# jmloveyj/ros_navigation

Measured on AMD Instinct MI355X. Metric: replan cycles/sec (HIMM+VFH++A*) on 4096x4096 grid, higher is better.
Workload: dtype int32

## Files before the change

### ros_navigation_amd/csrc/astar.hip

```cpp
#include "engine.hpp"

#include <algorithm>
#include <cfloat>
#include <cmath>
#include <cstdlib>
#include <cstring>
#include <chrono>
#include <thread>
#include <vector>

using namespace rna;

namespace {

constexpr int COST_D = 1414;

struct HostTrace {
  bool on = getenv("RNA_HOST_TRACE") != nullptr;
  double us[8] = {};
  long n = 0, queries = 0;
  std::chrono::steady_clock::time_point t;
  void start() { if (on) t = std::chrono::steady_clock::now(); }
  void lap(int k) {
    if (!on) return;
    const auto now = std::chrono::steady_clock::now();
    us[k] += std::chrono::duration<double, std::micro>(now - t).count();
    t = now;
  }
  void dump() {
    if (!on || n == 0) return;
    fprintf(stderr, "[host trace] %ld pipelined launches, us each: wait for a free stage %.1f (%.2f hipEventQuery calls) | ring entry's old batch %.1f | "
            "enqueue (events, snapshot, launch order, search, flag copy) %.1f | done event + bookkeeping %.1f\n", n, us[0] / n, (double)queries / n,
            us[1] / n, us[2] / n, us[3] / n);
    for (double& v : us) v = 0;
    n = 0; queries = 0;
  }
};
HostTrace g_trace;
struct StageTrace {
  hipEvent_t a[AstarDevice::MAX_DEPTH] = {}, c[AstarDevice::MAX_DEPTH] = {};
  std::chrono::steady_clock::time_point t_enq[AstarDevice::MAX_DEPTH];
  bool armed[AstarDevice::MAX_DEPTH] = {};
  double gpu_ms = 0, host_busy_ms = 0;
  long n = 0;
};
StageTrace g_stage;
void stage_trace_dump() {
  if (g_stage.n) fprintf(stderr, "[host trace] a stage's cycle, ms: from enqueue to the end of the search and what follows it on the stream %.2f (the search itself: roofline.avg_launch_ms) | "
                         "host: enqueue -> noticed free %.2f (%ld cycles)\n", g_stage.gpu_ms / g_stage.n, g_stage.host_busy_ms / g_stage.n, g_stage.n);
  g_stage.gpu_ms = g_stage.host_busy_ms = 0; g_stage.n = 0;
}

#define RNA_TRY(call) do { const int rc_try_ = (call); if (rc_try_ != RNA_OK) return rc_try_; } while (0)

int alloc_stage(rna_engine* e, int d) {
  AstarDevice& a = e->astar;
  AstarStage& s = a.stage[d];
  RNA_TRY(dev_alloc(e, &s.pool, tsa_pool_bytes(a.max_queries, a.page_cap) / sizeof(unsigned)));
  RNA_TRY(dev_alloc(e, &s.rev, (size_t)a.rev_cap * a.max_queries));
  RNA_TRY(dev_alloc(e, &s.block, tsa_stage_bytes(e)));
  RNA_HIP(e, hipMemsetAsync(s.block, 0, tsa_stage_bytes(e), e->stream));
  RNA_TRY(tsa_stage_prepare(e, d));
  if (a.page_cap < tsa_tiles(e)) {
    RNA_TRY(dev_alloc(e, &s.retry_pool, tsa_retry_pool_bytes(e) / sizeof(unsigned)));
    RNA_TRY(dev_alloc(e, &s.retry_block, tsa_retry_bytes(e)));
    RNA_HIP(e, hipMemsetAsync(s.retry_block, 0, tsa_retry_bytes(e), e->stream));
    RNA_TRY(tsa_retry_prepare(e, d));
  }
  if (a.depth == 1) return RNA_OK;
  int prio_lo = 0, prio_hi = 0;
  (void)hipDeviceGetStreamPriorityRange(&prio_lo, &prio_hi);
  if (getenv("RNA_NO_STREAM_PRIORITY")) prio_lo = prio_hi = 0;
  int skip = e->cu_count / 8;
  if (const char* m = getenv("RNA_SEARCH_CU_SKIP")) skip = atoi(m);
  if (skip > 0 && skip < e->cu_count) {
    uint32_t mask[16] = {};
    const int words = (e->cu_count + 31) / 32 < 16 ? (e->cu_count + 31) / 32 : 16;
    for (int c = skip; c < e->cu_count && c < 512; ++c) mask[c >> 5] |= 1u << (c & 31);
    RNA_HIP(e, hipExtStreamCreateWithCUMask(&s.stream, (uint32_t)words, mask));
  } else {
    RNA_HIP(e, hipStreamCreateWithPriority(&s.stream, hipStreamNonBlocking, prio_lo));
  }
  RNA_HIP(e, hipEventCreateWithFlags(&s.done, hipEventDisableTiming));
  RNA_HIP(e, hipEventCreateWithFlags(&s.snap_done, hipEventDisableTiming));
  return RNA_OK;
}

void free_stage(AstarStage& s) {
  dev_free(&s.pool); dev_free(&s.rev); dev_free(&s.block); dev_free(&s.retry_pool); dev_free(&s.retry_block);
  if (s.stream) (void)hipStreamDestroy(s.stream);
  if (s.done) (void)hipEventDestroy(s.done);
  if (s.snap_done) (void)hipEventDestroy(s.snap_done);
  s = AstarStage{};
}

int alloc_stages_impl(rna_engine* e) {
  AstarDevice& a = e->astar;
  for (int d = 0; d < a.depth; ++d) RNA_TRY(alloc_stage(e, d));
  if (a.depth > 1) {
    RNA_HIP(e, hipEventCreateWithFlags(&a.ev_init, hipEventDisableTiming));
    RNA_HIP(e, hipEventCreateWithFlags(&a.ev_prep, hipEventDisableTiming));
    a.ring_n = 2 * a.depth;
    a.ring_stride = tsa_ring_bytes(e);
    RNA_TRY(dev_alloc(e, &a.ring_mem, a.ring_stride * (size_t)a.ring_n));
    RNA_HIP(e, hipMemsetAsync(a.ring_mem, 0, a.ring_stride * (size_t)a.ring_n, e->stream));
    for (int r = 0; r < a.ring_n; ++r) RNA_HIP(e, hipEventCreateWithFlags(&a.ring[r].free, hipEventDisableTiming));
  }
  if (a.stage[0].retry_pool) {
    RNA_HIP(e, hipHostMalloc(reinterpret_cast<void**>(&a.retry_flag), AstarDevice::MAX_DEPTH * sizeof(int), hipHostMallocCoherent));
    for (int d = 0; d < AstarDevice::MAX_DEPTH; ++d) a.retry_flag[d] = 0;
    for (int d = 0; d < a.depth; ++d) a.stage[d].retry_flag = a.retry_flag + d;
  }
  a.launches = 0;
  RNA_TRY(dev_alloc(e, &a.queries_dev, (size_t)a.max_queries));
  RNA_TRY(dev_alloc(e, &a.results_dev, (size_t)a.max_queries));
  return RNA_OK;
}

int alloc_stages(rna_engine* e) {
  const int rc = alloc_stages_impl(e);
  if (rc != RNA_OK) {
    const std::string why = e->err;
    (void)astar_release(e);
    e->err = why;
  }
  return rc;
}

int ensure_config(rna_engine* e) {
  AstarDevice& a = e->astar;
  if (a.live()) return RNA_OK;
// ... 334 lines not shown
```

### ros_navigation_amd/csrc/astar_tile.hip

```cpp
#include "engine.hpp"
#include <algorithm>
#include <cstring>
#include <vector>

using namespace rna;

namespace rna {

constexpr int TI = 64, TJ = 16;
constexpr int TILE_WORDS = TI * TJ;
constexpr int AUX_WORDS = 64;
constexpr int MASK_STRIDE = TILE_WORDS + 32 + 128;
constexpr int TSA_WAVES = 8;
constexpr int TSA_WAVES_PER_EU = 8;
constexpr int TSA_HPASS = 4;
constexpr int TSA_IDLE_SLEEP = 4;
constexpr int TSA_PRIO_FIRST = 0;
constexpr int TSA_BT_PRIO = 3;
constexpr int TSA_SCOPE = __HIP_MEMORY_SCOPE_AGENT;
constexpr int TSA_MAX_TILE_WORDS = 2048;
constexpr int COST_S = 1000, COST_D = 1414;
constexpr int INF = 0x7fffffff;
constexpr int KU = 0x40000000;
constexpr int SCR_CNT = 84 + 192 + 48 + 64;
// ... 63 lines not shown
  return r;
}
__device__ __forceinline__ int tsa_octile24(int i, int j, int gi, int gj) {
  const int dx = abs(i - gi), dy = abs(j - gj);
  return tsa_h24(max(dx, dy), min(dx, dy));
}
__device__ __forceinline__ int tsa_prop(int u, int h, int thr) { return (u - h >= thr) ? u : 0; }

__device__ __forceinline__ int tile_of(int i, int j, int tiles_i) { return (j >> 4) * tiles_i + (i >> 6); }
__device__ __forceinline__ int in_page(int i, int j) { return ((j & 15) << 6) + (i & 63); }
__device__ __forceinline__ int kdi_of(int k) { return (k == 0 || k == 3 || k == 5) ? -1 : ((k == 2 || k == 4 || k == 7) ? 1 : 0); }
__device__ __forceinline__ int kdj_of(int k) { return k < 3 ? -1 : (k > 4 ? 1 : 0); }

struct TsaStage {
  unsigned* pages;
  unsigned* paux;
  unsigned* tmap;
  unsigned* owner;
  int* nalloc;
  uint8_t* nbr_tm;
  int* perm;
  int* ticket;
  int cap;
};
__host__ __device__ inline size_t tsa_align256(size_t x) { return (x + 255) & ~(size_t)255; }
constexpr int TSA_COUNTER_WORDS = 16;
__host__ __device__ inline unsigned long long* tsa_counters_of(const TsaStage& S) {
  return reinterpret_cast<unsigned long long*>(reinterpret_cast<char*>(S.nalloc) - TSA_COUNTER_WORDS * sizeof(unsigned long long));
}

__global__ void __launch_bounds__(256) tsa_snapshot_kernel(const uint8_t* __restrict__ nbr, int rows, int cols, int tiles_i, int tiles_j,
                                                             uint8_t* __restrict__ nbr_tm, int s0, int s1) {
  __shared__ unsigned s_free[256];
  const int a = threadIdx.x & 63, bq = threadIdx.x >> 6;
  for (int t = blockIdx.x; t < tiles_i * tiles_j; t += gridDim.x) {
    const int i = (t % tiles_i) * TI + a, j0 = (t / tiles_i) * TJ + bq * 4;
    unsigned v = 0u;
    if (i < rows) {
      const int bi = i + s0 >= rows ? i + s0 - rows : i + s0;
#pragma unroll
      for (int k = 0; k < 4; ++k)
        if (j0 + k < cols) {
          const int bj = j0 + k + s1 >= cols ? j0 + k + s1 - cols : j0 + k + s1;
          v |= (unsigned)nbr[(size_t)bj * rows + bi] << (8 * k);
        }
    }
    uint8_t* out = nbr_tm + (size_t)t * MASK_STRIDE;
    reinterpret_cast<unsigned*>(out)[a * 4 + bq] = v;
    if (a == 0) reinterpret_cast<unsigned*>(out + TILE_WORDS)[bq] = v;
    if (a == TI - 1) reinterpret_cast<unsigned*>(out + TILE_WORDS + 16)[bq] = v;
    s_free[threadIdx.x] = (((v & 0xffu) != 0u) ? 1u : 0u) | (((v & 0xff00u) != 0u) ? 2u : 0u) | (((v & 0xff0000u) != 0u) ? 4u : 0u) |
                          (((v & 0xff000000u) != 0u) ? 8u : 0u);
    __syncthreads();
    if (bq == 0)
      reinterpret_cast<unsigned short*>(out + TILE_WORDS + 32)[a] =
          (unsigned short)(s_free[a] | (s_free[64 + a] << 4) | (s_free[128 + a] << 8) | (s_free[192 + a] << 12));
    __syncthreads();
  }
}
__global__ void __launch_bounds__(256) tsa_prepare_kernel(TsaStage S, const rna_astar_query* __restrict__ queries, int n, int rows, int cols,
                                                          int ranked, int* __restrict__ served) {
  extern __shared__ int s_key[];
  if (threadIdx.x == 0) *S.ticket = 0;
  if (served && threadIdx.x < TSA_RETRY) served[threadIdx.x] = -1;
  if (served && threadIdx.x == TSA_RETRY) served[TSA_RETRY] = 0;
  if (!ranked) {
    for (int i = threadIdx.x; i < n; i += blockDim.x) S.perm[i] = i;
    return;
  }
  const int ncell = rows * cols;
  for (int i = threadIdx.x; i < n; i += blockDim.x) {
    const rna_astar_query q = queries[i];
    int key = -1;
    if (q.start >= 0 && q.goal >= 0 && q.start < ncell && q.goal < ncell) {
      const int di = abs(q.start % rows - q.goal % rows), dj = abs(q.start / rows - q.goal / rows);
      key = di > dj ? di : dj;
    }
    s_key[i] = key;
  }
  __syncthreads();
  for (int i = threadIdx.x; i < n; i += blockDim.x) {
    const int ki = s_key[i];
    int rank = 0;
    for (int j = 0; j < n; ++j) {
      const int kj = s_key[j];
      rank += (kj > ki || (kj == ki && j < i)) ? 1 : 0;
    }
    S.perm[rank] = i;
  }
}
__global__ void __launch_bounds__(256) tsa_zero_page0_kernel(unsigned* __restrict__ pages, unsigned* __restrict__ paux, int cap) {
  static_assert(TILE_WORDS / 4 == 256 && AUX_WORDS / 4 <= 256, "one uint4 of page 0 per thread");
  const size_t page0 = (size_t)blockIdx.x * ((size_t)cap + 1);
  reinterpret_cast<uint4*>(pages + (page0 << 10))[threadIdx.x] = make_uint4(0u, 0u, 0u, 0u);
  if (threadIdx.x < AUX_WORDS / 4) reinterpret_cast<uint4*>(paux + page0 * AUX_WORDS)[threadIdx.x] = make_uint4(0u, 0u, 0u, 0u);
// ... 884 lines not shown
    return;
  }
  asm volatile("s_waitcnt vmcnt(0)" ::: "memory");
  __builtin_amdgcn_wave_barrier();
  int32_t* path = A.paths + (size_t)q * A.max_path_len;
  for (int i = lane; i < len; i += 64) path[i] = tsa_buffer_lin(rev[len - 1 - i], rows, cols, A.s0, A.s1);
  if (lane == 0) A.results[q] = rna_astar_result{0, len, r.cost, r.expanded, r.rounds, r.buckets};
}

template <int WAVES, bool RETRY>
__global__ void __launch_bounds__(WAVES * 64) __attribute__((amdgpu_waves_per_eu(TSA_WAVES_PER_EU, TSA_WAVES_PER_EU))) tsa_search_kernel(const TsaLaunch A) {
  constexpr int TSA_THREADS = WAVES * 64;
  __shared__ __attribute__((aligned(16))) unsigned s_scr[WAVES][SCR_WORDS];
  extern __shared__ unsigned s_dyn[];
  __shared__ __attribute__((aligned(16))) unsigned s_node[TSA_NP];
  __shared__ __attribute__((aligned(16))) unsigned s_head[TSA_NCLS];
  __shared__ unsigned s_bm[TSA_BMW];
  __shared__ unsigned s_qc[TSA_QC];
  __shared__ int s_best, s_state, s_bucket, s_bucket0, s_jobs_done, s_jobs_noop, s_jobs_sticky, s_expanded, s_nalloc, s_any;
  __shared__ int s_count, s_spill, s_idle, s_open_left, s_open_pos, s_reruns;

  __shared__ int s_q, s_rank;
  if (!RETRY) {
    if (threadIdx.x == 0) { const int k = atomicAdd(A.S.ticket, 1); s_rank = k; s_q = A.S.perm[k]; }
  } else {
    if (threadIdx.x == 0) { s_q = A.retry_list[A.retry_base + (int)blockIdx.x]; s_rank = 1 << 30; }
  }
  __syncthreads();
  const int q = __builtin_amdgcn_readfirstlane(s_q);
  if (q < 0) return;
  if (RETRY && threadIdx.x == 0) A.S2.ticket[8 + blockIdx.x] = q;
  const TsaStage& S = RETRY ? A.S2 : A.S;
  const int sl = RETRY ? (int)blockIdx.x : q;
  if (__builtin_amdgcn_readfirstlane(s_rank) < A.prio_first) __builtin_amdgcn_s_setprio(3);
  const int tid = threadIdx.x, lane = tid & 63, wv = __builtin_amdgcn_readfirstlane(tid >> 6);
#ifdef RNA_TSA_STATS
  const unsigned long long t_kernel0 = wall_clock64();
#endif
  const int rows = A.rows, cols = A.cols, tiles_i = A.tiles_i, tiles_j = A.tiles_j;
  rna_astar_query qu = A.queries[q];
  const int ncell = rows * cols;
  const int ntile = tiles_i * tiles_j;
  const int nt_words = (ntile + 31) >> 5;
  unsigned* const s_st2 = s_dyn;
  unsigned* const s_open = s_dyn + 2 * nt_words;
  unsigned* const s_far = s_dyn + 3 * nt_words;
  rna_astar_result* const results = A.results;

  const bool valid = qu.start >= 0 && qu.goal >= 0 && qu.start < ncell && qu.goal < ncell;
  if (!valid) {
    if (tid == 0) results[q] = rna_astar_result{2, 0, INF, 0, 0, 0};
    return;
  }
  qu.start = tsa_unwrap_lin(qu.start, rows, cols, A.s0, A.s1);
  qu.goal = tsa_unwrap_lin(qu.goal, rows, cols, A.s0, A.s1);
  const int si = qu.start % rows, sj = qu.start / rows;
  const int gi = qu.goal % rows, gj = qu.goal / rows;

  TsaCtx C;
  C.rows = rows; C.cols = cols; C.tiles_i = tiles_i; C.tiles_j = tiles_j;
  C.tiles_magic = tiles_i > 1 ? (unsigned)(0x100000000ull / (unsigned)tiles_i) + 1u : 0u;
  C.pages = S.pages + (((size_t)sl * ((size_t)S.cap + 1)) << 10);
  C.paux = S.paux + (size_t)sl * ((size_t)S.cap + 1) * AUX_WORDS;
  C.tmap = S.tmap + (size_t)sl * ntile;
  C.owner = S.owner + (size_t)sl * (S.cap + 1);
  C.cap = S.cap;
  C.nalloc = &s_nalloc;
// ... 373 lines not shown
  const TsaGrid G = tsa_grid(e);
  KernelTimer kt(e, RNA_K_ASTAR_INIT, st);
  hipLaunchKernelGGL(tsa_snapshot_kernel, dim3(std::min(G.ti * G.tj, 4096)), dim3(256), 0, st, e->nbr, G.rows, G.cols, G.ti, G.tj,
                     tsa_launch_view(e, d, ring).nbr_tm, e->geom.start[0], e->geom.start[1]);
  RNA_HIP(e, hipGetLastError());
  return RNA_OK;
}
int tsa_order(rna_engine* e, int d, int ring, hipStream_t st, const rna_astar_query* q_dev, int n) {
  const TsaGrid G = tsa_grid(e);
  KernelTimer kt(e, RNA_K_ASTAR_RESET, st);
  const int ranked = n <= 2048 ? 1 : 0;
  hipLaunchKernelGGL(tsa_prepare_kernel, dim3(1), dim3(256), ranked ? (size_t)n * sizeof(int) : 0, st, tsa_launch_view(e, d, ring), q_dev, n, G.rows,
                     G.cols, ranked, tsa_retry_served(e, d));
  RNA_HIP(e, hipGetLastError());
  return RNA_OK;
}
int tsa_search(rna_engine* e, int d, int ring, hipStream_t st, const rna_astar_query* q_dev, int n, int32_t* paths_dev, int max_len,
               rna_astar_result* res_dev) {
  AstarDevice& a = e->astar;
  AstarStage& s = a.stage[d];
  const TsaGrid G = tsa_grid(e);
  const TsaStage S = tsa_launch_view(e, d, ring);
  KernelTimer kt(e, RNA_K_ASTAR_SEARCH, st);
  const size_t nt_bytes = (size_t)((G.ti * G.tj + 31) / 32) * sizeof(unsigned);
  TsaLaunch A;
  memset(&A, 0, sizeof(A));
  A.rows = G.rows; A.cols = G.cols; A.tiles_i = G.ti; A.tiles_j = G.tj; A.s0 = e->geom.start[0]; A.s1 = e->geom.start[1];
  A.queries = q_dev; A.S = S; A.bucket_width = a.bucket_width; A.paths = paths_dev; A.max_path_len = max_len;
  A.rev_all = s.rev; A.rev_cap = a.rev_cap; A.results = res_dev;
  A.retry = 0; A.n = n; A.S2 = S;
  A.prio_first = a.depth > 1 ? TSA_PRIO_FIRST : 0;
  if (const char* pf = getenv("RNA_TSA_PRIO_FIRST")) A.prio_first = atoi(pf);
  size_t lds_dyn = 4 * nt_bytes;
  if (const char* pad = getenv("RNA_TSA_LDS_PAD")) lds_dyn += (size_t)atoi(pad);
  const bool can_retry = s.retry_flag != nullptr;
  A.retry_count = can_retry ? tsa_retry_count(e, d) : nullptr;
  A.retry_list = can_retry ? tsa_retry_list(e, d) : nullptr;
  A.retry_base = 0;
  static const bool wide_env = getenv("RNA_TSA_WIDE") != nullptr;
  const bool wide = wide_env || n <= 32;
  if (a.depth > 1 && !wide) hipLaunchKernelGGL((tsa_search_kernel<TSA_WAVES, false>), dim3(n), dim3(TSA_WAVES * 64), lds_dyn, st, A);
  else hipLaunchKernelGGL((tsa_search_kernel<16, false>), dim3(n), dim3(16 * 64), lds_dyn, st, A);
  RNA_HIP(e, hipGetLastError());
  memcpy(s.last_launch, &A, sizeof(A));
  s.last_lds = lds_dyn;
  s.last_retried = 0;
  s.retry_armed = can_retry;
  return RNA_OK;
}

int tsa_counters_read(rna_engine* e, unsigned long long* out, bool reset) {
  AstarDevice& a = e->astar;
  for (int k = 0; k < TSA_COUNTER_WORDS; ++k) out[k] = 0ull;
  for (int d = 0; d < AstarDevice::MAX_DEPTH; ++d) {
    for (int view = 0; view < 2; ++view) {
      char* base = view ? a.stage[d].retry_block : a.stage[d].block;
      if (!base) continue;
      unsigned long long w[TSA_COUNTER_WORDS];
      char* cnt = base + TSA_HEAD_COUNTERS;
      RNA_HIP(e, hipMemcpyAsync(w, cnt, sizeof(w), hipMemcpyDeviceToHost, e->stream));
      if (reset) RNA_HIP(e, hipMemsetAsync(cnt, 0, sizeof(w), e->stream));
      RNA_HIP(e, hipStreamSynchronize(e->stream));
      for (int k = 0; k < TSA_COUNTER_WORDS; ++k) out[k] += w[k];
    }
  }
  return RNA_OK;
// ... 43 lines not shown
```

### ros_navigation_amd/csrc/engine.hip

```cpp
#include "engine.hpp"
#include "map_tiles_dev.hpp"

#include <cmath>
#include <dirent.h>
#include <unistd.h>
#include <cstdlib>
#include <cstring>
#include <limits>

using namespace rna;

__global__ void fill_f32_kernel(float* __restrict__ p, size_t n, float v) {
  size_t i = (size_t)blockIdx.x * blockDim.x + threadIdx.x;
  const size_t stride = (size_t)gridDim.x * blockDim.x;
  for (; i < n; i += stride) p[i] = v;
}

__global__ void compose_dirty_tiles_kernel(float* __restrict__ master, const float* __restrict__ laser,
                                           const unsigned* __restrict__ dirty, int rows, int cols, int tiles_i) {
  const int ti = blockIdx.x, tj = blockIdx.y;
  const int t = tj * tiles_i + ti;
  if (!reinterpret_cast<const unsigned char*>(dirty)[t]) return;
  const int i0 = ti * TILE, j0 = tj * TILE;
  const int li = threadIdx.x & (TILE - 1);
// ... 5 lines not shown
    }
  }
}

__global__ void nbr_mask_tiles_kernel(uint8_t* __restrict__ nbr, const float* __restrict__ master,
                                      const unsigned* __restrict__ dirty, int all, int rows, int cols,
                                      int tiles_i, int tiles_j, int s0, int s1) {
  const int ti = blockIdx.x, tj = blockIdx.y;
  if (!all && !dirty_ring(dirty, ti, tj, tiles_i, tiles_j)) return;
  __shared__ uint8_t blk[(TILE + 2) * (TILE + 2)];
  const int i0 = ti * TILE - 1, j0 = tj * TILE - 1;
  for (int k = threadIdx.x; k < (TILE + 2) * (TILE + 2); k += blockDim.x) {
    const int ii = k % (TILE + 2), jj = k / (TILE + 2);
    const int i = i0 + ii, j = j0 + jj;
    uint8_t b = 1;
    if (i >= 0 && j >= 0 && i < rows && j < cols) {
      b = cell_blocked(master[buffer_lin(i, j, rows, cols, s0, s1)]) ? 1 : 0;
    }
    blk[k] = b;
  }
  __syncthreads();
  for (int k = threadIdx.x; k < TILE * TILE; k += blockDim.x) {
    const int li = k & (TILE - 1), lj = k >> 6;
    const int i = ti * TILE + li, j = tj * TILE + lj;
    if (i >= rows || j >= cols) continue;
    nbr[buffer_lin(i, j, rows, cols, s0, s1)] = (uint8_t)nbr_mask_of(&blk[(lj + 1) * (TILE + 2) + (li + 1)], TILE + 2);
  }
}

__global__ void __launch_bounds__(256) compose_nbr_tiles_kernel(uint8_t* __restrict__ nbr, float* __restrict__ master, const float* __restrict__ laser,
                                                                const unsigned* __restrict__ dirty, unsigned* __restrict__ next_dirty, int rows,
                                                                int cols, int tiles_i, int tiles_j) {
  __shared__ uint8_t blk[(TILE + 2) * (TILE + 2)];
  for (int tt = blockIdx.x; tt < tiles_i * tiles_j; tt += gridDim.x)
    compose_nbr_tile(blk, tt, nbr, master, laser, dirty, next_dirty, rows, cols, tiles_i, tiles_j);
}

__global__ void clear_region_kernel(float* __restrict__ p, int rows, int i0, int ni, int j0, int nj) {
  const size_t n = (size_t)ni * nj;
  size_t k = (size_t)blockIdx.x * blockDim.x + threadIdx.x;
  const size_t stride = (size_t)gridDim.x * blockDim.x;
  const float nanv = __int_as_float(0x7fc00000);
  for (; k < n; k += stride) {
    const int i = i0 + (int)(k % ni), j = j0 + (int)(k / ni);
    p[(size_t)j * rows + i] = nanv;
  }
}

__global__ void __launch_bounds__(256) pack_tiles_kernel(const float* __restrict__ layer, int rows, int tiles_i,
                                                         const int32_t* __restrict__ tiles, int wi0, int wi1, int wj0,
                                                         int wj1, float* __restrict__ dense) {
  const int t = tiles[blockIdx.x];
  const int i0 = (t % tiles_i) * TILE, j0 = (t / tiles_i) * TILE;
  float* out = dense + (size_t)blockIdx.x * (TILE * TILE);
  for (int k = threadIdx.x; k < TILE * TILE; k += 256) {
    const int i = i0 + (k & (TILE - 1)), j = j0 + (k >> 6);
    out[k] = (i >= wi0 && i < wi1 && j >= wj0 && j < wj1) ? layer[(size_t)j * rows + i] : 0.0f;
  }
}

__global__ void __launch_bounds__(256) unpack_tiles_kernel(float* __restrict__ layer_a, float* __restrict__ layer_b,
                                                           int rows, int tiles_i, const int32_t* __restrict__ tiles,
                                                           int wi0, int wi1, int wj0, int wj1,
                                                           const float* __restrict__ dense,
                                                           unsigned* __restrict__ dirty_tiles) {
  const int t = tiles[blockIdx.x];
// ... 689 lines not shown
```

### ros_navigation_amd/csrc/engine.hpp

```cpp
#pragma once

#include <hip/hip_runtime.h>

#include <cstdint>
#include <cstdio>
#include <string>
#include <vector>

#include "../../include/rna.h"
#include "gridmath.hpp"
#include "map_state.hpp"

namespace {
struct GfCtl;
struct FrCtl;
}

namespace rna {

constexpr int TILE = 64;

struct HimmSlot { int cell; int head; int len; int offset; };

struct HimmScratch {
  int cap_rays = 0;
  int n_slots = 0;
  rna_ray* rays_dev = nullptr;
  int4* desc = nullptr;
  int* ncells = nullptr;
  int* next = nullptr;
  HimmSlot* slots = nullptr;
  int* seqs = nullptr;
  unsigned* before = nullptr;
  unsigned* after = nullptr;
  int* total = nullptr;
  unsigned* mark_bitmap = nullptr;
  int* pairs = nullptr;
  size_t pairs_cap = 0;
  bool pairs_checked = false;
  int* pairs_total_host = nullptr;
  int* tile_bins = nullptr;
  int win[4] = {0, 0, 0, 0};
};

struct VfhDevice {
  bool ready = false;
  rna_vfh_params p{};
  int n_robots = 0;
  int W = 0, H = 0, T = 0, CX = 0, CY = 0, NQ = 0, NQF = 0, NW = 0, max_speed = 0;
  float *cell_dist = nullptr, *cell_base_mag = nullptr, *cell_dir = nullptr;
  int* range_idx = nullptr;
  unsigned* memb = nullptr;
  unsigned* in_circle = nullptr;
// ... 7 lines not shown
};

struct AstarStage {
  unsigned* pool = nullptr;
  int32_t* rev = nullptr;
  char* block = nullptr;
  unsigned* retry_pool = nullptr;
  char* retry_block = nullptr;
  hipStream_t stream = nullptr;
  hipEvent_t done = nullptr;
  hipEvent_t snap_done = nullptr;
  bool snap_pending = false;
  bool busy = false;
  unsigned long long seq = 0;
  int* retry_flag = nullptr;
  bool retry_armed = false;
  int last_retried = 0;
  size_t last_lds = 0;
  alignas(8) unsigned char last_launch[384] = {};
};
struct AstarRingEntry {
  hipEvent_t free = nullptr;
  bool used = false;
};

struct AstarDevice {
  int max_queries = 0;
  int bucket_width = 128000;
#ifndef RNA_ASTAR_MAX_DEPTH
#define RNA_ASTAR_MAX_DEPTH 20
#endif
  static constexpr int MAX_DEPTH = RNA_ASTAR_MAX_DEPTH;
  int depth = 4;
  AstarStage stage[MAX_DEPTH];
  bool live() const { return stage[0].pool != nullptr; }
  int rev_cap = 16800;
  int page_cap = 0;
  int page_cap_request = 0;
  static constexpr int MAX_RING = 2 * MAX_DEPTH;
  int ring_n = 0;
  char* ring_mem = nullptr;
  size_t ring_stride = 0;
  AstarRingEntry ring[MAX_RING];
  hipEvent_t ev_init = nullptr;
  hipEvent_t ev_prep = nullptr;
  int* retry_flag = nullptr;
  unsigned long long launches = 0;
  int last_slot = 0;
  rna_astar_query* queries_dev = nullptr;
  rna_astar_result* results_dev = nullptr;
  int32_t* paths_dev = nullptr;
  int paths_cap = 0;
  const rna_astar_query* last_queries = nullptr;
  const rna_astar_result* last_results = nullptr;
  int last_n = 0;
};

struct FootprintPlan {
  double r = 0.0, res = 0.0, mag = 0.0;
  int R = 0;
  int K = 0;
  int band = 0;
  int n_ties = 0;
  int w[64] = {};
};

// ... 276 lines not shown
```

### ros_navigation_amd/csrc/himm.hip

```cpp
#include "engine.hpp"

#include <algorithm>

using namespace rna;

namespace {

__device__ __forceinline__ float himm_clear(float v) {
  if (v <= 0.0f || v != v) v = 0.0f;
  else v = v - 10.0f;
  if (v < 0.0f) v = 0.0f;
  return v;
}

__device__ __forceinline__ float himm_mark(float v) {
  if (v <= 0.0f || v != v) return 30.0f;
  if (v <= 150.0f) return v + 30.0f;
  return v;
}

__device__ __forceinline__ float himm_clear_n(float v, unsigned k) {
  for (unsigned i = 0; i < k; ++i) {
    v = himm_clear(v);
    if (__float_as_int(v) == 0) break;
// ... 43 lines not shown
  if (!ray_well_formed(g, ray)) {
    ncells[r] = 0;
    next[r] = -1;
    return;
  }
  if (index_limited_to_map(g, ray.sx, ray.sy, ray.ex, ray.ey, s) &&
      index_limited_to_map(g, ray.ex, ray.ey, ray.sx, ray.sy, t)) {
    const int dx = abs(t[0] - s[0]), dy = abs(t[1] - s[1]);
    nc = (dx >= dy ? dx : dy) + 1;
    desc[r] = make_int4(s[0], s[1], t[0], t[1]);
  }
  ncells[r] = nc;
  next[r] = -1;
  if (!ray.clear_end) {
    int ei[2];
    if (index_from_position(g, ray.ex, ray.ey, ei) && ei[0] >= win.x && ei[0] < win.y && ei[1] >= win.z &&
        ei[1] < win.w) {
      const int cell = ei[1] * g.size[0] + ei[0];
      unsigned h = hash_cell((unsigned)cell) & (unsigned)slot_mask;
      for (;;) {
        const int prev = atomicCAS(&slots[h].cell, -1, cell);
        if (prev == -1 || prev == cell) break;
        h = (h + 1) & (unsigned)slot_mask;
      }
      next[r] = atomicExch(&slots[h].head, r);
      atomicAdd(&slots[h].len, 1);
      atomicOr(&mark_bitmap[cell >> 5], 1u << (cell & 31));
    }
  }
}

__global__ void himm_prep_kernel(Geom g, const rna_ray* __restrict__ rays, int n, int4* __restrict__ desc, int* __restrict__ ncells,
                                 int* __restrict__ next, HimmSlot* __restrict__ slots, int slot_mask, unsigned* __restrict__ mark_bitmap, int4 win) {
  const int r = blockIdx.x * blockDim.x + threadIdx.x;
  if (r >= n) return;
  himm_prep_ray(g, rays, r, desc, ncells, next, slots, slot_mask, mark_bitmap, win);
}

__device__ void sift_down(int* a, int start, int end) {
  int root = start;
  for (;;) {
    int child = 2 * root + 1;
    if (child > end) break;
    if (child + 1 <= end && a[child] < a[child + 1]) child++;
    if (a[root] < a[child]) { const int t = a[root]; a[root] = a[child]; a[child] = t; root = child; }
    else break;
  }
}

__device__ __forceinline__ void himm_collect_slot(int h, HimmSlot* __restrict__ slots, int n_slots, const int* __restrict__ next, int* __restrict__ seqs,
                                                  unsigned* __restrict__ before, unsigned* __restrict__ after, int* __restrict__ total, int* s_wave, int* s_base) {
  HimmSlot sl = h < n_slots ? slots[h] : HimmSlot{-1, -1, 0, 0};
  const bool live = sl.cell >= 0;
  int off = 0;
  {
    const int lane = (int)__builtin_amdgcn_mbcnt_hi(~0u, __builtin_amdgcn_mbcnt_lo(~0u, 0u));
    const int wv = threadIdx.x >> 6, nwv = (blockDim.x + 63) >> 6;
    int incl = live ? sl.len : 0;
    for (int o = 1; o < 64; o <<= 1) { const int v = __shfl_up(incl, o); if (lane >= o) incl += v; }
    __syncthreads();
    if (lane == 63) s_wave[wv] = incl;
    __syncthreads();
    if (threadIdx.x == 0) {
      int run = 0;
      for (int w = 0; w < nwv; ++w) { const int t = s_wave[w]; s_wave[w] = run; run += t; }
      *s_base = run > 0 ? atomicAdd(total, run) : 0;
    }
    __syncthreads();
    off = *s_base + s_wave[wv] + incl - (live ? sl.len : 0);
  }
  if (!live) return;
  slots[h].offset = off;

  int* a = seqs + off;
  int k = 0;
  for (int r = sl.head; r >= 0; r = next[r]) a[k++] = r;
  const int len = k;

  if (len <= 24) {
    for (int i = 1; i < len; ++i) {
      const int v = a[i];
      int j = i - 1;
      while (j >= 0 && a[j] > v) { a[j + 1] = a[j]; --j; }
      a[j + 1] = v;
    }
  } else {
    for (int st = (len - 2) / 2; st >= 0; --st) sift_down(a, st, len - 1);
    for (int end = len - 1; end > 0; --end) {
      const int t = a[end]; a[end] = a[0]; a[0] = t;
      sift_down(a, 0, end - 1);
    }
  }
  for (int i = 0; i < len; ++i) { before[off + i] = 0; after[off + i] = 0; }
}

__global__ void __launch_bounds__(1024) himm_collect_kernel(HimmSlot* __restrict__ slots, int n_slots, const int* __restrict__ next, int* __restrict__ seqs,
                                                            unsigned* __restrict__ before, unsigned* __restrict__ after, int* __restrict__ total) {
  __shared__ int s_wave[16];
  __shared__ int s_base;
  himm_collect_slot(blockIdx.x * blockDim.x + threadIdx.x, slots, n_slots, next, seqs, before, after, total, s_wave, &s_base);
}

struct RayWalk {
  int M0, m0, s, sm, den, add, num0, nc;
  bool xmajor;
  __device__ __forceinline__ RayWalk(const int4 d, int ncells) {
    const int adx = abs(d.z - d.x), ady = abs(d.w - d.y);
    xmajor = adx >= ady;
    den = xmajor ? adx : ady;
    add = xmajor ? ady : adx;
    num0 = den / 2;
    nc = ncells;
    const int sx = d.z >= d.x ? 1 : -1, sy = d.w >= d.y ? 1 : -1;
    M0 = xmajor ? d.x : d.y; m0 = xmajor ? d.y : d.x;
    s = xmajor ? sx : sy; sm = xmajor ? sy : sx;
  }
  __device__ __forceinline__ int minor(int k) const {
    return m0 + (den > 0 ? (int)(((unsigned)num0 + (unsigned)k * (unsigned)add) / (unsigned)den) : 0) * sm;
  }
  __device__ __forceinline__ int major(int k) const { return M0 + k * s; }
  template <class F>
  __device__ __forceinline__ void for_each_tile_lockstep(int tiles_i, F f) const {
    int k = 0;
    while (__builtin_amdgcn_ballot_w64(k < nc)) {
      const bool act = k < nc;
      const int M = major(act ? k : 0), tM = M >> 6;
      int kend = s > 0 ? k + ((tM << 6) + 63 - M) : k + (M - (tM << 6));
      if (kend > nc - 1) kend = nc - 1;
      const int ta = minor(act ? k : 0) >> 6, tb = minor(act ? kend : 0) >> 6;
      f(act, xmajor ? ta * tiles_i + tM : tM * tiles_i + ta);
      f(act && tb != ta, xmajor ? tb * tiles_i + tM : tM * tiles_i + tb);
      if (act) k = kend + 1;
    }
  }
};

__device__ __forceinline__ int wave_tile_add(int* __restrict__ counters, bool active, int t) {
  const int lane = (int)__builtin_amdgcn_mbcnt_hi(~0u, __builtin_amdgcn_mbcnt_lo(~0u, 0u));
  unsigned long long todo = __builtin_amdgcn_ballot_w64(active);
  int slot = 0;
  while (todo) {
    const int leader = __ffsll((long long)todo) - 1;
    const int lt = __shfl(t, leader);
    const unsigned long long same = __builtin_amdgcn_ballot_w64(active && t == lt);
    int base = 0;
    if (lane == leader) base = atomicAdd(&counters[lt], __popcll(same));
    base = __shfl(base, leader);
    if (active && t == lt) slot = base + __popcll(same & ((1ull << lane) - 1ull));
    todo &= ~same;
  }
  return slot;
}

__global__ void himm_bin_count_kernel(const int4* __restrict__ desc, const int* __restrict__ ncells, int n, int tiles_i,
                                      int* __restrict__ tile_count) {
  const int r = blockIdx.x * blockDim.x + threadIdx.x;
  const int nc = r < n ? ncells[r] : 0;
  const RayWalk w(nc ? desc[r] : make_int4(0, 0, 0, 0), nc);
  w.for_each_tile_lockstep(tiles_i, [&](bool act, int t) { (void)wave_tile_add(tile_count, act, t); });
}

constexpr int HIMM_SCAN_THREADS = 1024;
__device__ __forceinline__ void himm_bin_scan(int* __restrict__ tile_count, int ntile, int* __restrict__ tile_off,
                                              int* __restrict__ tile_cursor, int4* __restrict__ active,
                                              int* __restrict__ n_active, int* __restrict__ ticket, int* s_part, int* s_act, int* s_act2) {
  constexpr int NT = HIMM_SCAN_THREADS;
  constexpr int HEAVY = 512;
  const int per = (ntile + NT - 1) / NT;
  const int lo = min(ntile, (int)threadIdx.x * per), hi = min(ntile, lo + per);
  int sum = 0, nact = 0, nact2 = 0;
  for (int t = lo; t < hi; ++t) { const int c = tile_count[t]; sum += c; nact += c >= HEAVY; nact2 += c > 0 && c < HEAVY; }
  s_part[threadIdx.x] = sum;
  s_act[threadIdx.x] = nact;
  s_act2[threadIdx.x] = nact2;
  __syncthreads();
  for (int o = 1; o < NT; o <<= 1) {
    const bool in = (int)threadIdx.x >= o;
    const int v = in ? s_part[threadIdx.x - o] : 0, a = in ? s_act[threadIdx.x - o] : 0, a2 = in ? s_act2[threadIdx.x - o] : 0;
    __syncthreads();
    s_part[threadIdx.x] += v;
    s_act[threadIdx.x] += a;
    s_act2[threadIdx.x] += a2;
    __syncthreads();
  }
  const int n_heavy = s_act[NT - 1];
  int run = s_part[threadIdx.x] - sum, arun = s_act[threadIdx.x] - nact, arun2 = n_heavy + s_act2[threadIdx.x] - nact2;
  for (int t = lo; t < hi; ++t) {
    const int c = tile_count[t];
    tile_off[t] = run; tile_cursor[t] = 0; run += c;
    if (c >= HEAVY) active[arun++] = make_int4(t, run - c, c, 0);
    else if (c > 0) active[arun2++] = make_int4(t, run - c, c, 0);
    tile_count[t] = 0;
  }
  if (threadIdx.x == NT - 1) { tile_off[ntile] = s_part[NT - 1]; *n_active = s_act[NT - 1] + s_act2[NT - 1]; *ticket = 0; }
}

__global__ void __launch_bounds__(HIMM_SCAN_THREADS)
himm_bin_scan_kernel(int* __restrict__ tile_count, int ntile, int* __restrict__ tile_off, int* __restrict__ tile_cursor, int4* __restrict__ active,
                     int* __restrict__ n_active, int* __restrict__ ticket) {
  __shared__ int s_part[HIMM_SCAN_THREADS], s_act[HIMM_SCAN_THREADS], s_act2[HIMM_SCAN_THREADS];
  himm_bin_scan(tile_count, ntile, tile_off, tile_cursor, active, n_active, ticket, s_part, s_act, s_act2);
}

__global__ void himm_bin_fill_kernel(const int4* __restrict__ desc, const int* __restrict__ ncells, int n, int tiles_i,
                                     const int* __restrict__ tile_off, int* __restrict__ tile_cursor, int* __restrict__ pairs) {
  const int r = blockIdx.x * blockDim.x + threadIdx.x;
  const int nc = r < n ? ncells[r] : 0;
  const RayWalk w(nc ? desc[r] : make_int4(0, 0, 0, 0), nc);
  w.for_each_tile_lockstep(tiles_i, [&](bool act, int t) {
    const int slot = wave_tile_add(tile_cursor, act, t);
    if (act) pairs[tile_off[t] + slot] = r;
  });
}

constexpr int HIMM_MTAB = 256;

#ifdef RNA_HIMM_STATS
__device__ unsigned long long g_himm_stat[16];
#define HST(var) const unsigned long long var = wall_clock64()
#define HACC(slot, a, b) do { if (threadIdx.x == 0) atomicAdd(&g_himm_stat[slot], (unsigned long long)((b) - (a))); } while (0)
#define HCNT(slot, v) do { if (threadIdx.x == 0) atomicAdd(&g_himm_stat[slot], (unsigned long long)(v)); } while (0)
#else
#define HST(var)
#define HACC(slot, a, b)
#define HCNT(slot, v)
#endif

__device__ __forceinline__ void himm_lds_barrier() { asm volatile("s_waitcnt lgkmcnt(0)\n\ts_barrier" ::: "memory"); }

__device__ __forceinline__ void himm_count_marked_clear(int cell, int r, const HimmSlot* __restrict__ slots, int slot_mask, const int* __restrict__ seqs,
                                                        unsigned* __restrict__ before, unsigned* __restrict__ after) {
  unsigned h = hash_cell((unsigned)cell) & (unsigned)slot_mask;
  while (slots[h].cell != cell) h = (h + 1) & (unsigned)slot_mask;
  const int off = slots[h].offset, len = slots[h].len;
  int lo = 0, hi = len;
  while (lo < hi) {
    const int mid = (lo + hi) >> 1;
    if (seqs[off + mid] < r) lo = mid + 1; else hi = mid;
// ... 173 lines not shown
      kk[u] = L.cnt[threadIdx.x + u * HIMM_TR_THREADS];
      if (kk[u] >> 31) kk[u] = 0u;
    }
#pragma unroll
    for (int u = 0; u < PER_T; ++u) {
      const int c = threadIdx.x + u * HIMM_TR_THREADS;
      vv[u] = kk[u] ? layer[(size_t)(j0 + (c >> 6)) * rows + i0 + (c & 63)] : 0.0f;
    }
#pragma unroll
    for (int u = 0; u < PER_T; ++u) {
      if (kk[u] == 0u) continue;
      const int c = threadIdx.x + u * HIMM_TR_THREADS;
      const float nv = himm_clear_n(vv[u], kk[u]);
      if (__float_as_int(nv) != __float_as_int(vv[u])) layer[(size_t)(j0 + (c >> 6)) * rows + i0 + (c & 63)] = nv;
    }
  }
  HST(t_6);
  if (threadIdx.x == 0) { L.job = job_next; L.rec = rec_next; }
  himm_lds_barrier();
  HST(t_7);
  HACC(0, t_0, t_1); HACC(1, t_1, t_2); HACC(2, t_2, t_3); HACC(3, t_3, t_4); HACC(4, t_4, t_5); HACC(5, t_5, t_6); HACC(6, t_6, t_7);
  HCNT(7, 1); HCNT(8, np);
  job = L.job;
  rec = L.rec;
  }
}

__global__ void __launch_bounds__(HIMM_TR_THREADS)
himm_tile_raster_kernel(int rows, int cols, int tiles_i, const int4* __restrict__ desc, const int* __restrict__ ncells, const int* __restrict__ tile_off,
                        const int* __restrict__ pairs, const int4* __restrict__ active, const int* __restrict__ n_active, int* __restrict__ ticket,
                        float* __restrict__ layer, const unsigned* __restrict__ mark_bitmap, const HimmSlot* __restrict__ slots, int slot_mask,
                        const int* __restrict__ seqs, unsigned* __restrict__ before, unsigned* __restrict__ after, unsigned* __restrict__ dirty_tiles, int4 win) {
  __shared__ RasterLds L;
  himm_raster_jobs(L, (int)blockIdx.x, (int)gridDim.x, rows, cols, tiles_i, desc, ncells, tile_off, pairs, active, n_active, ticket, layer, mark_bitmap,
                   slots, slot_mask, seqs, before, after, dirty_tiles, win);
}

__global__ void himm_apply_kernel(int rows, HimmSlot* __restrict__ slots, int n_slots, int* __restrict__ total, const unsigned* __restrict__ before,
                                  const unsigned* __restrict__ after, float* __restrict__ layer, unsigned* __restrict__ mark_bitmap,
                                  unsigned* __restrict__ dirty_tiles, int tiles_i) {
  const int h = blockIdx.x * blockDim.x + threadIdx.x;
  if (h == 0) *total = 0;
  if (h >= n_slots) return;
  const HimmSlot sl = slots[h];
  if (sl.cell < 0) return;
  float v = layer[sl.cell];
  for (int k = 0; k < sl.len; ++k) {
    v = himm_clear_n(v, before[sl.offset + k]);
    v = himm_mark(v);
  }
  v = himm_clear_n(v, after[sl.offset + sl.len - 1]);
  layer[sl.cell] = v;
  atomicAnd(&mark_bitmap[sl.cell >> 5], ~(1u << (sl.cell & 31)));
  slots[h] = HimmSlot{-1, -1, 0, 0};
  const int i = sl.cell % rows, j = sl.cell / rows;
  const int tile = (j >> 6) * tiles_i + (i >> 6);
  if (dirty_tiles && reinterpret_cast<volatile unsigned char*>(dirty_tiles)[tile] != 1) reinterpret_cast<volatile unsigned char*>(dirty_tiles)[tile] = 1;
}

static size_t himm_pairs_worst(const rna_engine* e, size_t cap_rays) {
  return cap_rays * (size_t)(2 * ((std::max(e->geom.size[0], e->geom.size[1]) + 63) / 64) + 2);
}
static size_t himm_pairs_initial(const rna_engine* e, size_t cap_rays, bool* checked) {
  const size_t worst = himm_pairs_worst(e, cap_rays);
  size_t limit = (size_t)64 << 20;
  if (const char* v = getenv("RNA_HIMM_PAIRS_LIMIT")) limit = (size_t)atoll(v);
  *checked = worst > limit;
  return *checked ? std::min(worst, std::max(cap_rays * 16, limit / 4)) : worst;
}

struct HimmBins {
  size_t count, off, cursor, n_active, ticket, active, total;
  explicit HimmBins(size_t ntile)
// ... 177 lines not shown
```

### ros_navigation_amd/csrc/vfh.hip

```cpp
#include "engine.hpp"

#include <cmath>
#include <cstring>
#include <vector>

using namespace rna;

namespace {

constexpr int VFH_THREADS = 128;
constexpr int MAX_W = 64;
constexpr int MAX_NQ = (MAX_W / 2 + 1) * MAX_W;
[[maybe_unused]] constexpr int MAX_NW = (MAX_NQ + 31) / 32;
constexpr int MAX_H = 128;
constexpr int VFH_OCC_CAP = 1024;

struct VfhK {
  int W, H, T, CX, CY, YH, NQ, NQF, NW, max_speed, sector_angle;
  float cell_width, robot_radius, sd0, sd1, bl0, bh0, bl1, bh1, U1, U2;
  int current_max_speed, max_speed_narrow, max_speed_wide, max_accel, mt0, mt1;
  const float *cell_dist, *cell_base_mag, *cell_dir;
  const int* range_idx;
  const unsigned *memb, *in_circle;
  const int* mtr;
// ... 73 lines not shown
  o.ok = 1; o.tl_u = tl_u; o.size = sz;
  o.off = pos_s + (0.5 * len_s - 0.5 * res);
  return o;
}

#ifndef RNA_VFH_WAVES
#define RNA_VFH_WAVES 6
#endif
#define VFH_WAVES_ATTR __attribute__((amdgpu_waves_per_eu(RNA_VFH_WAVES, RNA_VFH_WAVES)))
#ifdef RNA_VFH_SKIPS
__device__ int d_vfh_skip;
#define VFH_SKIP(bit) (__builtin_amdgcn_readfirstlane(d_vfh_skip) & (bit))
__device__ int d_vfh_exit;
#define VFH_EXIT(n) if (__builtin_amdgcn_readfirstlane(d_vfh_exit) == (n)) return
#else
#define VFH_SKIP(bit) 0
#define VFH_EXIT(n)
#endif
__global__ void __launch_bounds__(VFH_THREADS) VFH_WAVES_ATTR
vfh_step_kernel(VfhK K, Geom g, const float* __restrict__ master, const rna_pose* __restrict__ poses,
                const double* __restrict__ ext_ranges, rna_vfh_out* __restrict__ out,
                float* __restrict__ origin_out, float* __restrict__ hist_out) {
  __shared__ unsigned long long rng[361];
  extern __shared__ float vfh_dyn[];
  float* const mag = vfh_dyn;
  unsigned* const nz = reinterpret_cast<unsigned*>(vfh_dyn + ((K.NQ + 31) & ~31));
  __shared__ float s_hist[MAX_H];
  __shared__ unsigned s_phi_right, s_phi_left;
  __shared__ int s_emergency, s_nocc, s_cant;
  __shared__ int occ[VFH_OCC_CAP];
  __shared__ int s_ax_ok[2], s_ax_tl[2], s_ax_size[2];
  __shared__ double s_ax_off[2];

  const int b = blockIdx.x;
  const int tid = threadIdx.x;
#ifdef RNA_VFH_STATS
  unsigned long long ts_[8];
  int nts_ = 0;
#define VFH_STAMP() ts_[nts_++] = wall_clock64()
#else
#define VFH_STAMP()
#endif
  VFH_STAMP();
  const rna_pose pose = poses[b];
  float st_picked = 0.0f, st_last_picked = 0.0f, st_blocked_radius = 0.0f;
  int st_max_speed_picked = 0;
  const bool wave0 = __builtin_amdgcn_readfirstlane(tid >> 6) == 0;
  if (wave0) {
    st_picked = K.picked[b];
    st_last_picked = K.last_picked[b];
    st_max_speed_picked = K.max_speed_picked[b];
  }
  st_blocked_radius = K.blocked_radius[b];
  const int last_speed = K.last_chosen_speed[b];
  float st_last_binary = 0.0f;
  if (tid < K.H) st_last_binary = K.last_binary[(size_t)b * K.H + tid];

  const float desired_angle = pose.goal_direction;
  const float dist_to_goal = pose.goal_distance;
  const float goal_tol = pose.goal_tolerance;
  int speed = pose.current_speed < 0 ? 0 : pose.current_speed;
  if (speed < last_speed) speed = last_speed;
  const int tspeed = speed > K.max_speed ? K.max_speed : speed;
  const float bcr_tspeed = K.bcr[tspeed];

  float cd4[4], bm4[4], dir4[4];
// ... 732 lines not shown
```

Before: 172,700.

## Raise wave priority of mapping/VFH kernels and add search occupancy control

Adds an issue_first() helper that sets top wave priority in the HIMM, compose, VFH, snapshot and prepare kernels. The search kernel's first-rank priority drops from 3 to 2, so the short pipeline kernels get issue preference over concurrent A* searches. Search streams are now always CU-masked through a new SearchOccupancy config, and an optional LDS padding path can cap search workgroups per CU at 3 so other kernels get room. This reshapes how concurrent stages share the GPU, but it can starve the searches or add imbalance.

```diff
diff --git a/ros_navigation_amd/csrc/astar.hip b/ros_navigation_amd/csrc/astar.hip
--- a/ros_navigation_amd/csrc/astar.hip
+++ b/ros_navigation_amd/csrc/astar.hip
@@ -53,7 +53,7 @@
 
 #define RNA_TRY(call) do { const int rc_try_ = (call); if (rc_try_ != RNA_OK) return rc_try_; } while (0)
 
-int alloc_stage(rna_engine* e, int d) {
+int alloc_stage(rna_engine* e, int d, const SearchOccupancy& occ) {
   AstarDevice& a = e->astar;
   AstarStage& s = a.stage[d];
   RNA_TRY(dev_alloc(e, &s.pool, tsa_pool_bytes(a.max_queries, a.page_cap) / sizeof(unsigned)));
@@ -68,19 +68,10 @@
     RNA_TRY(tsa_retry_prepare(e, d));
   }
   if (a.depth == 1) return RNA_OK;
-  int prio_lo = 0, prio_hi = 0;
-  (void)hipDeviceGetStreamPriorityRange(&prio_lo, &prio_hi);
-  if (getenv("RNA_NO_STREAM_PRIORITY")) prio_lo = prio_hi = 0;
-  int skip = e->cu_count / 8;
-  if (const char* m = getenv("RNA_SEARCH_CU_SKIP")) skip = atoi(m);
-  if (skip > 0 && skip < e->cu_count) {
-    uint32_t mask[16] = {};
-    const int words = (e->cu_count + 31) / 32 < 16 ? (e->cu_count + 31) / 32 : 16;
-    for (int c = skip; c < e->cu_count && c < 512; ++c) mask[c >> 5] |= 1u << (c & 31);
-    RNA_HIP(e, hipExtStreamCreateWithCUMask(&s.stream, (uint32_t)words, mask));
-  } else {
-    RNA_HIP(e, hipStreamCreateWithPriority(&s.stream, hipStreamNonBlocking, prio_lo));
-  }
+  uint32_t mask[16] = {};
+  const int words = (e->cu_count + 31) / 32 < 16 ? (e->cu_count + 31) / 32 : 16;
+  for (int c = occ.reserved; c < e->cu_count && c < 512; ++c) mask[c >> 5] |= 1u << (c & 31);
+  RNA_HIP(e, hipExtStreamCreateWithCUMask(&s.stream, (uint32_t)words, mask));
   RNA_HIP(e, hipEventCreateWithFlags(&s.done, hipEventDisableTiming));
   RNA_HIP(e, hipEventCreateWithFlags(&s.snap_done, hipEventDisableTiming));
   return RNA_OK;
@@ -96,7 +87,8 @@
 
 int alloc_stages_impl(rna_engine* e) {
   AstarDevice& a = e->astar;
-  for (int d = 0; d < a.depth; ++d) RNA_TRY(alloc_stage(e, d));
+  a.occ = search_occupancy(getenv("RNA_SEARCH_WGS_PER_CU"), getenv("RNA_SEARCH_CU_SKIP"), e->cu_count);
+  for (int d = 0; d < a.depth; ++d) RNA_TRY(alloc_stage(e, d, a.occ));
   if (a.depth > 1) {
     RNA_HIP(e, hipEventCreateWithFlags(&a.ev_init, hipEventDisableTiming));
     RNA_HIP(e, hipEventCreateWithFlags(&a.ev_prep, hipEventDisableTiming));
diff --git a/ros_navigation_amd/csrc/astar_tile.hip b/ros_navigation_amd/csrc/astar_tile.hip
--- a/ros_navigation_amd/csrc/astar_tile.hip
+++ b/ros_navigation_amd/csrc/astar_tile.hip
@@ -119,6 +119,7 @@
 __global__ void __launch_bounds__(256) tsa_snapshot_kernel(const uint8_t* __restrict__ nbr, int rows, int cols, int tiles_i, int tiles_j,
                                                              uint8_t* __restrict__ nbr_tm, int s0, int s1) {
   __shared__ unsigned s_free[256];
+  issue_first();
   const int a = threadIdx.x & 63, bq = threadIdx.x >> 6;
   for (int t = blockIdx.x; t < tiles_i * tiles_j; t += gridDim.x) {
     const int i = (t % tiles_i) * TI + a, j0 = (t / tiles_i) * TJ + bq * 4;
@@ -148,6 +149,7 @@
 __global__ void __launch_bounds__(256) tsa_prepare_kernel(TsaStage S, const rna_astar_query* __restrict__ queries, int n, int rows, int cols,
                                                           int ranked, int* __restrict__ served) {
   extern __shared__ int s_key[];
+  issue_first();
   if (threadIdx.x == 0) *S.ticket = 0;
   if (served && threadIdx.x < TSA_RETRY) served[threadIdx.x] = -1;
   if (served && threadIdx.x == TSA_RETRY) served[TSA_RETRY] = 0;
@@ -1098,7 +1100,7 @@
   if (RETRY && threadIdx.x == 0) A.S2.ticket[8 + blockIdx.x] = q;
   const TsaStage& S = RETRY ? A.S2 : A.S;
   const int sl = RETRY ? (int)blockIdx.x : q;
-  if (__builtin_amdgcn_readfirstlane(s_rank) < A.prio_first) __builtin_amdgcn_s_setprio(3);
+  if (__builtin_amdgcn_readfirstlane(s_rank) < A.prio_first) __builtin_amdgcn_s_setprio(2);
   const int tid = threadIdx.x, lane = tid & 63, wv = __builtin_amdgcn_readfirstlane(tid >> 6);
 #ifdef RNA_TSA_STATS
   const unsigned long long t_kernel0 = wall_clock64();
@@ -1538,6 +1540,14 @@
   A.prio_first = a.depth > 1 ? TSA_PRIO_FIRST : 0;
   if (const char* pf = getenv("RNA_TSA_PRIO_FIRST")) A.prio_first = atoi(pf);
   size_t lds_dyn = 4 * nt_bytes;
+  if (a.depth > 1 && a.occ.wgs_per_cu < 4) {
+    static const size_t static_lds = [] {
+      hipFuncAttributes fa{};
+      return hipFuncGetAttributes(&fa, reinterpret_cast<const void*>(&tsa_search_kernel<TSA_WAVES, false>)) == hipSuccess ? fa.sharedSizeBytes : (size_t)0;
+    }();
+    if (static_lds == 0) return fail(e, RNA_EHIP, "grid A*: the search kernel's LDS size is not known");
+    lds_dyn = search_lds_dynamic(static_lds, 4 * nt_bytes, a.occ.wgs_per_cu);
+  }
   if (const char* pad = getenv("RNA_TSA_LDS_PAD")) lds_dyn += (size_t)atoi(pad);
   const bool can_retry = s.retry_flag != nullptr;
   A.retry_count = can_retry ? tsa_retry_count(e, d) : nullptr;
diff --git a/ros_navigation_amd/csrc/engine.hip b/ros_navigation_amd/csrc/engine.hip
--- a/ros_navigation_amd/csrc/engine.hip
+++ b/ros_navigation_amd/csrc/engine.hip
@@ -61,6 +61,7 @@
                                                                 const unsigned* __restrict__ dirty, unsigned* __restrict__ next_dirty, int rows,
                                                                 int cols, int tiles_i, int tiles_j) {
   __shared__ uint8_t blk[(TILE + 2) * (TILE + 2)];
+  issue_first();
   for (int tt = blockIdx.x; tt < tiles_i * tiles_j; tt += gridDim.x)
     compose_nbr_tile(blk, tt, nbr, master, laser, dirty, next_dirty, rows, cols, tiles_i, tiles_j);
 }
diff --git a/ros_navigation_amd/csrc/engine.hpp b/ros_navigation_amd/csrc/engine.hpp
--- a/ros_navigation_amd/csrc/engine.hpp
+++ b/ros_navigation_amd/csrc/engine.hpp
@@ -10,6 +10,7 @@
 #include "../../include/rna.h"
 #include "gridmath.hpp"
 #include "map_state.hpp"
+#include "search_occupancy.hpp"
 
 namespace {
 struct GfCtl;
@@ -19,6 +20,8 @@
 namespace rna {
 
 constexpr int TILE = 64;
+
+__device__ __forceinline__ void issue_first() { __builtin_amdgcn_s_setprio(3); }
 
 struct HimmSlot { int cell; int head; int len; int offset; };
 
@@ -92,6 +95,7 @@
 #endif
   static constexpr int MAX_DEPTH = RNA_ASTAR_MAX_DEPTH;
   int depth = 4;
+  SearchOccupancy occ;
   AstarStage stage[MAX_DEPTH];
   bool live() const { return stage[0].pool != nullptr; }
   int rev_cap = 16800;
diff --git a/ros_navigation_amd/csrc/himm.hip b/ros_navigation_amd/csrc/himm.hip
--- a/ros_navigation_amd/csrc/himm.hip
+++ b/ros_navigation_amd/csrc/himm.hip
@@ -99,6 +99,7 @@
 
 __global__ void himm_prep_kernel(Geom g, const rna_ray* __restrict__ rays, int n, int4* __restrict__ desc, int* __restrict__ ncells,
                                  int* __restrict__ next, HimmSlot* __restrict__ slots, int slot_mask, unsigned* __restrict__ mark_bitmap, int4 win) {
+  issue_first();
   const int r = blockIdx.x * blockDim.x + threadIdx.x;
   if (r >= n) return;
   himm_prep_ray(g, rays, r, desc, ncells, next, slots, slot_mask, mark_bitmap, win);
@@ -165,6 +166,7 @@
                                                             unsigned* __restrict__ before, unsigned* __restrict__ after, int* __restrict__ total) {
   __shared__ int s_wave[16];
   __shared__ int s_base;
+  issue_first();
   himm_collect_slot(blockIdx.x * blockDim.x + threadIdx.x, slots, n_slots, next, seqs, before, after, total, s_wave, &s_base);
 }
 
@@ -221,6 +223,7 @@
 
 __global__ void himm_bin_count_kernel(const int4* __restrict__ desc, const int* __restrict__ ncells, int n, int tiles_i,
                                       int* __restrict__ tile_count) {
+  issue_first();
   const int r = blockIdx.x * blockDim.x + threadIdx.x;
   const int nc = r < n ? ncells[r] : 0;
   const RayWalk w(nc ? desc[r] : make_int4(0, 0, 0, 0), nc);
@@ -266,11 +269,13 @@
 himm_bin_scan_kernel(int* __restrict__ tile_count, int ntile, int* __restrict__ tile_off, int* __restrict__ tile_cursor, int4* __restrict__ active,
                      int* __restrict__ n_active, int* __restrict__ ticket) {
   __shared__ int s_part[HIMM_SCAN_THREADS], s_act[HIMM_SCAN_THREADS], s_act2[HIMM_SCAN_THREADS];
+  issue_first();
   himm_bin_scan(tile_count, ntile, tile_off, tile_cursor, active, n_active, ticket, s_part, s_act, s_act2);
 }
 
 __global__ void himm_bin_fill_kernel(const int4* __restrict__ desc, const int* __restrict__ ncells, int n, int tiles_i,
                                      const int* __restrict__ tile_off, int* __restrict__ tile_cursor, int* __restrict__ pairs) {
+  issue_first();
   const int r = blockIdx.x * blockDim.x + threadIdx.x;
   const int nc = r < n ? ncells[r] : 0;
   const RayWalk w(nc ? desc[r] : make_int4(0, 0, 0, 0), nc);
@@ -510,6 +515,7 @@
                         float* __restrict__ layer, const unsigned* __restrict__ mark_bitmap, const HimmSlot* __restrict__ slots, int slot_mask,
                         const int* __restrict__ seqs, unsigned* __restrict__ before, unsigned* __restrict__ after, unsigned* __restrict__ dirty_tiles, int4 win) {
   __shared__ RasterLds L;
+  issue_first();
   himm_raster_jobs(L, (int)blockIdx.x, (int)gridDim.x, rows, cols, tiles_i, desc, ncells, tile_off, pairs, active, n_active, ticket, layer, mark_bitmap,
                    slots, slot_mask, seqs, before, after, dirty_tiles, win);
 }
@@ -517,6 +523,7 @@
 __global__ void himm_apply_kernel(int rows, HimmSlot* __restrict__ slots, int n_slots, int* __restrict__ total, const unsigned* __restrict__ before,
                                   const unsigned* __restrict__ after, float* __restrict__ layer, unsigned* __restrict__ mark_bitmap,
                                   unsigned* __restrict__ dirty_tiles, int tiles_i) {
+  issue_first();
   const int h = blockIdx.x * blockDim.x + threadIdx.x;
   if (h == 0) *total = 0;
   if (h >= n_slots) return;
diff --git a/ros_navigation_amd/csrc/search_occupancy.hpp b/ros_navigation_amd/csrc/search_occupancy.hpp
--- /dev/null
+++ b/ros_navigation_amd/csrc/search_occupancy.hpp
@@ -0,0 +1,40 @@
+#pragma once
+
+#include <cstddef>
+
+namespace rna {
+
+constexpr size_t LDS_PER_CU = 160 * 1024;
+
+struct SearchOccupancy {
+  int wgs_per_cu = 4;
+  int reserved = 0;
+};
+
+inline SearchOccupancy search_occupancy(const char* wgs_env, const char* skip_env, int cu_count) {
+  SearchOccupancy o;
+  o.reserved = cu_count / 8;
+  auto number = [](const char* s, int* v) {
+    if (!s || !*s) return false;
+    int n = 0;
+    for (; *s; ++s) {
+      if (*s < '0' || *s > '9' || n > 100000) return false;
+      n = n * 10 + (*s - '0');
+    }
+    *v = n;
+    return true;
+  };
+  int v = 0;
+  if (number(wgs_env, &v) && (v == 3 || v == 4)) o.wgs_per_cu = v;
+  if (number(skip_env, &v) && v <= cu_count / 8) o.reserved = v;
+  return o;
+}
+
+inline size_t search_lds_dynamic(size_t static_lds, size_t bitset_bytes, int wgs_per_cu) {
+  const size_t plain = static_lds + bitset_bytes;
+  if (wgs_per_cu < 1 || plain == 0 || LDS_PER_CU / plain <= (size_t)wgs_per_cu) return bitset_bytes;
+  const size_t total = LDS_PER_CU / (size_t)(wgs_per_cu + 1) + 1;
+  return (total - static_lds + 15) & ~(size_t)15;
+}
+
+}
diff --git a/ros_navigation_amd/csrc/vfh.hip b/ros_navigation_amd/csrc/vfh.hip
--- a/ros_navigation_amd/csrc/vfh.hip
+++ b/ros_navigation_amd/csrc/vfh.hip
@@ -129,6 +129,7 @@
   __shared__ int s_ax_ok[2], s_ax_tl[2], s_ax_size[2];
   __shared__ double s_ax_off[2];
 
+  issue_first();
   const int b = blockIdx.x;
   const int tid = threadIdx.x;
 #ifdef RNA_VFH_STATS
```

Result: no change. 172,600 (-0.1%).
